# gitvicky/CP-PRE

Measured on AMD Instinct MI355X. Metric: residual-cells/s (PRE eval+calibrate), higher is better.
Workload: dtype f32

## Files before the change

### cp_pre_amd/csrc/calib.hip

```cpp
#include "common.h"

#pragma clang fp contract(off)

namespace {

__global__ void __launch_bounds__(256) absdiff_kernel(const float *__restrict__ a, const float *__restrict__ b,
                                                      float *__restrict__ out, long long n)
{
    const bool vec = !(((uintptr_t)a | (uintptr_t)out | (uintptr_t)(b ? b : a)) & 15);
    long long done = 0;
    if (vec) {
        const long long n4 = n / 4;
        const float4 *a4 = reinterpret_cast<const float4 *>(a);
        const float4 *b4 = reinterpret_cast<const float4 *>(b);
        float4 *o4 = reinterpret_cast<float4 *>(out);
        for (long long blk = blockIdx.x; blk * 1024 < n4; blk += gridDim.x) {
            const long long i = blk * 1024 + threadIdx.x;
            float4 v[4], w[4];
#pragma unroll
            for (int u = 0; u < 4; ++u)
                if (i + u * 256 < n4) v[u] = a4[i + u * 256];
            if (b) {
#pragma unroll
                for (int u = 0; u < 4; ++u)
                    if (i + u * 256 < n4) {
                        w[u] = b4[i + u * 256];
                        v[u] = make_float4(v[u].x - w[u].x, v[u].y - w[u].y, v[u].z - w[u].z, v[u].w - w[u].w);
                    }
            }
#pragma unroll
            for (int u = 0; u < 4; ++u)
                if (i + u * 256 < n4) o4[i + u * 256] = make_float4(fabsf(v[u].x), fabsf(v[u].y), fabsf(v[u].z), fabsf(v[u].w));
        }
        done = n4 * 4;
    }
    const long long stride = (long long)gridDim.x * blockDim.x;
    const long long tid = (long long)blockIdx.x * blockDim.x + threadIdx.x;
    for (long long i = done + tid; i < n; i += stride) out[i] = fabsf(b ? a[i] - b[i] : a[i]);
}

__global__ void __launch_bounds__(256) std_axis0_kernel(const float *__restrict__ a, const float *__restrict__ b,
                                                        int n, long long M, float eps, float *__restrict__ mod)
{
    const long long c = (long long)blockIdx.x * blockDim.x + threadIdx.x;
    if (c >= M) return;
    const float *pa = a + c, *pb = b ? b + c : nullptr;
    float s = 0.f;
#pragma unroll 16
    for (int i = 0; i < n; ++i) {
        const float v = pb ? pa[(long long)i * M] - pb[(long long)i * M] : pa[(long long)i * M];
        s = s + v;
    }
    const float mean = s / (float)n;
    float acc = 0.f;
#pragma unroll 16
    for (int i = 0; i < n; ++i) {
        const float v = pb ? pa[(long long)i * M] - pb[(long long)i * M] : pa[(long long)i * M];
        const float d = v - mean;
        const float dd = d * d;
        acc = acc + dd;
    }
    mod[c] = sqrtf(acc / (float)n) + eps;
}

__global__ void __launch_bounds__(256) moments_kernel(const float *__restrict__ a, const float *__restrict__ b,
                                                      int n, long long M, long long ld, int rows_per_split,
                                                      double *__restrict__ sum, double *__restrict__ sumsq)
{
    const long long c = (long long)blockIdx.x * blockDim.x + threadIdx.x;
    if (c >= M) return;
    const int i0 = blockIdx.y * rows_per_split;
    const int i1 = min(n, i0 + rows_per_split);
    double s = 0.0, q = 0.0;
#pragma unroll 8
    for (int i = i0; i < i1; ++i) {
        float v = a[(long long)i * ld + c];
        if (b) v = v - b[(long long)i * ld + c];
        const double d = (double)v;
        s += d;
        q += d * d;
    }
    if (gridDim.y == 1) { sum[c] += s; sumsq[c] += q; }
    else { atomicAdd(&sum[c], s); atomicAdd(&sumsq[c], q); }
}

constexpr int MS_TMAX = 16;
#ifndef MS_WANT1
#define MS_WANT1 1024
#endif
#ifndef MS_STAGE
#define MS_STAGE 1
#endif
__device__ __forceinline__ unsigned int wave_max_u32_to_lane63(unsigned int v)
{
#define PRE_DPP_MAX(ctrl, rows)                                                                                                 \
    v = max(v, (unsigned int)__builtin_amdgcn_update_dpp(0, (int)v, ctrl, rows, 0xf, true))
    PRE_DPP_MAX(0x111, 0xf);
    PRE_DPP_MAX(0x112, 0xf);
    PRE_DPP_MAX(0x114, 0xf);
    PRE_DPP_MAX(0x118, 0xf);
    PRE_DPP_MAX(0x142, 0xa);
    PRE_DPP_MAX(0x143, 0xc);
#undef PRE_DPP_MAX
    return v;
}

template <int O>
__device__ __forceinline__ unsigned int dpp_xor(unsigned int x)
{
    if constexpr (O == 1) return (unsigned int)__builtin_amdgcn_update_dpp(0, (int)x, 0xB1, 0xf, 0xf, true);
    else if constexpr (O == 2) return (unsigned int)__builtin_amdgcn_update_dpp(0, (int)x, 0x4E, 0xf, 0xf, true);
    else if constexpr (O == 8) return (unsigned int)__builtin_amdgcn_update_dpp(0, (int)x, 0x128, 0xf, 0xf, true);
    else {
        const int t = __builtin_amdgcn_update_dpp(0, (int)x, 0x104, 0xf, 0x5, false);
        return (unsigned int)__builtin_amdgcn_update_dpp(t, (int)x, 0x114, 0xf, 0xa, false);
    }
}

typedef unsigned int ms_u32x2 __attribute__((ext_vector_type(2)));
template <int US, int H>
__device__ __forceinline__ void ms_butterfly(unsigned int (&m)[US], int lane)
{
    if constexpr (H >= 1) {
        constexpr int width = 64 * H / US;
#pragma unroll
        for (int k = 0; k < H; ++k) {
            if constexpr (width == 32) {
                const ms_u32x2 r = __builtin_amdgcn_permlane32_swap(m[k], m[H + k], false, false);
                m[k] = max(r.x, r.y);
            } else if constexpr (width == 16) {
                const ms_u32x2 r = __builtin_amdgcn_permlane16_swap(m[k], m[H + k], false, false);
                m[k] = max(r.x, r.y);
            } else {
                const bool up = lane & width;
                const unsigned int mine = up ? m[H + k] : m[k], send = up ? m[k] : m[H + k];
                m[k] = max(mine, dpp_xor<width>(send));
            }
        }
        ms_butterfly<US, H / 2>(m, lane);
    }
}

__device__ __forceinline__ float ms_cell(const float *p, unsigned int cb, unsigned int plane_bytes)
{
    const __amdgpu_buffer_rsrc_t r = __builtin_amdgcn_make_buffer_rsrc(const_cast<float *>(p), 0, plane_bytes, 0x00020000);
    return __uint_as_float(__builtin_amdgcn_raw_buffer_load_b32(r, (int)cb, 0, 0));
}

template <int TCH, int US, bool FULL>
__device__ __forceinline__ void ms_load(const float *__restrict__ au, unsigned int c, long long row_stride, long long plane, int i, int nt,
                                        float (&v)[US][TCH])
{
#pragma unroll
    for (int u = 0; u < US; ++u)
#pragma unroll
        for (int t = 0; t < TCH; ++t)
            v[u][t] = ms_cell(au + ((i + u) * row_stride + (FULL || TCH == 1 || t < nt ? t : nt - 1) * plane), c, (unsigned int)plane * 4u);
}

struct MsStage { unsigned int (*m)[17]; unsigned int *row0; long long nseg_left; };
template <int TCH, int US, bool FULL>
__device__ __forceinline__ void ms_use(const float (&v)[US][TCH], int i, int nt, bool scored, double (&s)[TCH], double (&q)[TCH],
                                       unsigned int *__restrict__ seg, long long seg_stride, const MsStage *stage = nullptr)
{
    unsigned int m[US];
#pragma unroll
    for (int u = 0; u < US; ++u) {
        int mp = 0;
        unsigned int mn = 0u;
#pragma unroll
        for (int t = 0; t < TCH; ++t) {
            const float x = (FULL || TCH == 1 || t < nt) ? v[u][t] : 0.f;
            const double d = (double)x;
            s[t] += d;
            q[t] = __builtin_fma(d, d, q[t]);
            mp = max(mp, (int)__float_as_uint(x));
            mn = max(mn, __float_as_uint(x));
        }
        m[u] = max((unsigned int)mp, mn & 0x7fffffffu);
        m[u] = scored ? m[u] : 0u;
    }
    const int lane = threadIdx.x & 63;
    if constexpr (US == 1) {
        m[0] = wave_max_u32_to_lane63(m[0]);
        if (lane == 63 && seg) seg[i * seg_stride] = m[0];
    } else {
        ms_butterfly<US, US / 2>(m, lane);
        if constexpr (64 / US > 8) m[0] = max(m[0], dpp_xor<8>(m[0]));
        if constexpr (64 / US > 4) m[0] = max(m[0], dpp_xor<4>(m[0]));
        m[0] = max(m[0], dpp_xor<2>(m[0]));
        m[0] = max(m[0], dpp_xor<1>(m[0]));
        if (US == 16 && stage) {
            if ((lane & 3) == 0) stage->m[threadIdx.x >> 6][lane >> 2] = m[0];
            __syncthreads();
            if (threadIdx.x < 256) {
                const int smp = (int)(threadIdx.x >> 4), sg = (int)(threadIdx.x & 15);
                if (sg < stage->nseg_left) stage->row0[(i + smp) * seg_stride + sg] = stage->m[sg][smp];
            }
            __syncthreads();
        } else if ((lane & (64 / US - 1)) == 0) seg[(i + lane / (64 / US)) * seg_stride] = m[0];
    }
}

template <int TCH, int US, bool FULL>
__device__ __forceinline__ void ms_samples(const float *__restrict__ au, unsigned int c, long long row_stride, long long plane, int i0, int i1,
                                           int nt, bool scored, double (&s)[TCH], double (&q)[TCH], unsigned int *__restrict__ seg,
                                           long long seg_stride, const MsStage *stage = nullptr)
{
    int i = i0;
    if constexpr (US == 1) {
        float va[1][TCH], vb[1][TCH];
        if (i < i1) ms_load<TCH, 1, FULL>(au, c, row_stride, plane, i, nt, va);
        for (; i < i1; i += 2) {
            ms_load<TCH, 1, FULL>(au, c, row_stride, plane, min(i + 1, i1 - 1), nt, vb);
            ms_use<TCH, 1, FULL>(va, i, nt, scored, s, q, seg, seg_stride);
            if (i + 1 >= i1) break;
            ms_load<TCH, 1, FULL>(au, c, row_stride, plane, min(i + 2, i1 - 1), nt, va);
            ms_use<TCH, 1, FULL>(vb, i + 1, nt, scored, s, q, seg, seg_stride);
        }
    } else {
        float v[US][TCH], w[US][TCH], v1[1][TCH];
        const int ilast = i0 + (i1 - i0) / US * US - US;
        if (i + US <= i1) ms_load<TCH, US, FULL>(au, c, row_stride, plane, i, nt, v);
        for (; i + US <= i1; i += 2 * US) {
            ms_load<TCH, US, FULL>(au, c, row_stride, plane, min(i + US, ilast), nt, w);
            ms_use<TCH, US, FULL>(v, i, nt, scored, s, q, seg, seg_stride, stage);
            if (i + 2 * US > i1) { i += US; break; }
            ms_load<TCH, US, FULL>(au, c, row_stride, plane, min(i + 2 * US, ilast), nt, v);
            ms_use<TCH, US, FULL>(w, i + US, nt, scored, s, q, seg, seg_stride, stage);
        }
        for (; i < i1; ++i) {
            ms_load<TCH, 1, FULL>(au, c, row_stride, plane, i, nt, v1);
            ms_use<TCH, 1, FULL>(v1, i, nt, scored, s, q, seg, seg_stride);
        }
    }
}

template <int TCH, int US>
__global__ void __launch_bounds__(US == 16 && MS_STAGE ? 1024 : 256)
moments_segmax_kernel(const float *__restrict__ a, long long row_stride, int n, int T, int X,
                                                             int Y, int cx, int cy, int rows_per_split, double *__restrict__ sum,
                                                             double *__restrict__ sumsq, unsigned int *__restrict__ segmax)
{
    const long long plane = (long long)X * Y, cl = (long long)blockIdx.x * blockDim.x + threadIdx.x;
    if (!(US == 16 && MS_STAGE) && (cl & ~63LL) >= plane) return;
    const bool live = cl < plane;
    const long long c = live ? cl : plane - 1;
    const int x = (int)(c / Y), y = (int)(c - (long long)x * Y);
    const long long nseg = (plane + 63) / 64;
    const bool scored = live && x >= cx && x < X - cx && y >= cy && y < Y - cy;
    const int i0 = blockIdx.y * rows_per_split, i1 = min(n, i0 + rows_per_split);
    const int tc = blockIdx.z, TC = gridDim.z, t0 = tc * MS_TMAX, nt = min(TCH, T - t0);
    const float *au = a + (long long)t0 * plane;
    const long long seg_stride = (long long)TC * nseg;
    unsigned int *seg = segmax + (long long)tc * nseg + (cl >> 6);
    double s[TCH], q[TCH];
#pragma unroll
    for (int t = 0; t < TCH; ++t) s[t] = q[t] = 0.0;
    const unsigned int cb = (unsigned int)c * 4u;
    __shared__ unsigned int stage_m[US == 16 ? 16 : 1][17];
    MsStage st{stage_m, segmax + (long long)tc * nseg + (long long)blockIdx.x * (blockDim.x >> 6),
               nseg - (long long)blockIdx.x * (blockDim.x >> 6)};
    const MsStage *stage = (US == 16 && MS_STAGE) ? &st : nullptr;
    if (US == 16 && MS_STAGE && (cl & ~63LL) >= plane) seg = nullptr;
    if (nt == TCH) ms_samples<TCH, US, true>(au, cb, row_stride, plane, i0, i1, nt, scored, s, q, seg, seg_stride, stage);
    else ms_samples<TCH, US, false>(au, cb, row_stride, plane, i0, i1, nt, scored, s, q, seg, seg_stride, stage);
    sum += (long long)t0 * plane + c;
    sumsq += (long long)t0 * plane + c;
#pragma unroll
    for (int t = 0; t < TCH; ++t)
        if (t < nt && live) {
            if (gridDim.y == 1) { sum[t * plane] += s[t]; sumsq[t * plane] += q[t]; }
            else { atomicAdd(&sum[t * plane], s[t]); atomicAdd(&sumsq[t * plane], q[t]); }
        }
}

__global__ void __launch_bounds__(256) std_from_moments_kernel(const double *__restrict__ sum, const double *__restrict__ sumsq,
                                                               double n_total, long long M, float eps, float *__restrict__ mod)
{
    const long long c = (long long)blockIdx.x * blockDim.x + threadIdx.x;
    if (c >= M) return;
    const double mean = sum[c] / n_total;
    double var = sumsq[c] / n_total - mean * mean;
    var = var < 0.0 ? 0.0 : var;
    mod[c] = (float)sqrt(var) + eps;
}

__device__ __forceinline__ float wave_max(float v)
{
#pragma unroll
    for (int o = 32; o > 0; o >>= 1) v = fmaxf(v, __shfl_xor(v, o));
    return v;
}

constexpr int JS_RB = 32;
#ifndef JS_TARGET_CELLS
#define JS_TARGET_CELLS 65536
#endif
__device__ __forceinline__ void js_update(float av, float sv, float &m, float &thr, bool &nan)
{
    if (!(av <= thr * sv) || sv < 1.17549435e-38f) {
        const float q = av / sv;
        if (q != q) nan = true;
        else if (q > m) { m = q; thr = m * 0.99999905f; }
    }
}

__global__ void __launch_bounds__(256) joint_score_kernel(const float *__restrict__ a, const float *__restrict__ b,
                                                          const float *__restrict__ mod, int T, int X, int Y,
                                                          int ct, int cx, int cy, int groups, int smp_fastest,
                                                          const unsigned int *__restrict__ only, float *__restrict__ scores)
{
    const long long plane = (long long)X * Y, vol = plane * T;
    const int smp = smp_fastest ? blockIdx.x : blockIdx.y;
    const unsigned int cblk = smp_fastest ? blockIdx.y : blockIdx.x;
    if (only && !only[smp]) return;
    const float *pa = a + smp * vol, *pb = b ? b + smp * vol : nullptr;
    const long long nrows = (long long)T * X;
    const bool vec = (Y % 4 == 0) && !(((uintptr_t)a | (uintptr_t)mod | (uintptr_t)(b ? b : a)) & 15);
    __shared__ unsigned int rowmask;
    __shared__ float red[4];
    float m = 0.f, thr = 0.f;
    bool any = false, nan = false;
    for (int gi = 0; gi < groups; ++gi) {
    const long long r0 = ((long long)cblk * groups + gi) * JS_RB;
    if (r0 >= nrows) break;
    __syncthreads();
    if (threadIdx.x < 64) {
        const long long r = r0 + threadIdx.x;
        bool ok = threadIdx.x < JS_RB && r < nrows;
        if (ok) {
            const int t = (int)(r / X), x = (int)(r % X);
            ok = !(t < ct || t >= T - ct || x < cx || x >= X - cx);
        }
        const unsigned long long bm = __ballot(ok);
        if (threadIdx.x == 0) rowmask = (unsigned int)bm;
    }
    __syncthreads();
    const unsigned int rows = rowmask;
    any = any || rows != 0u;
    if (rows && vec) {
        const int Y4 = Y / 4, dr = 256 / Y4, dy = 256 % Y4;
        int row = threadIdx.x / Y4, y4 = threadIdx.x % Y4;
        while (row < JS_RB) {
            if ((rows >> row) & 1u) {
                const long long o = (r0 + row) * Y + 4 * y4;
                float4 v = *reinterpret_cast<const float4 *>(pa + o);
                if (pb) { const float4 w = *reinterpret_cast<const float4 *>(pb + o); v = make_float4(v.x - w.x, v.y - w.y, v.z - w.z, v.w - w.w); }
                const float4 sg = *reinterpret_cast<const float4 *>(mod + o);
                const float av[4] = {fabsf(v.x), fabsf(v.y), fabsf(v.z), fabsf(v.w)};
                const float sv[4] = {sg.x, sg.y, sg.z, sg.w};
                const int y = 4 * y4;
#pragma unroll
                for (int k = 0; k < 4; ++k)
                    if (y + k >= cy && y + k < Y - cy) js_update(av[k], sv[k], m, thr, nan);
            }
            y4 += dy;
            row += dr;
            if (y4 >= Y4) { y4 -= Y4; ++row; }
        }
    } else if (rows) {
        const int dr = 256 / Y, dy = 256 % Y;
        int row = threadIdx.x / Y, y = threadIdx.x % Y;
        while (row < JS_RB) {
            if (((rows >> row) & 1u) && y >= cy && y < Y - cy) {
                const long long o = (r0 + row) * Y + y;
                float v = pa[o];
                if (pb) v -= pb[o];
                js_update(fabsf(v), mod[o], m, thr, nan);
            }
            y += dy;
            row += dr;
            if (y >= Y) { y -= Y; ++row; }
        }
    }
    }
    m = wave_max(m);
    if (__ballot(nan)) m = __uint_as_float(0x7fc00000u);
    if ((threadIdx.x & 63) == 0) red[threadIdx.x >> 6] = m;
    __syncthreads();
    if (threadIdx.x == 0 && any) {
        const unsigned int u = max(max(__float_as_uint(red[0]), __float_as_uint(red[1])),
                                   max(__float_as_uint(red[2]), __float_as_uint(red[3])));
        atomicMax(reinterpret_cast<unsigned int *>(scores) + smp, u);
    }
}

constexpr int JSF_CELLS = 8192;
__global__ void __launch_bounds__(256) joint_score_flat_kernel(const float *__restrict__ a, const float *__restrict__ b,
                                                               const float *__restrict__ mod, int T, int X, int Y, int ct,
                                                               int cx, int cy, const unsigned int *__restrict__ only,
                                                               float *__restrict__ scores)
{
    const long long vol = (long long)T * X * Y;
    const int smp = blockIdx.x;
    if (only && !only[smp]) return;
    const float4 *pa = reinterpret_cast<const float4 *>(a + smp * vol);
    const float4 *pb = b ? reinterpret_cast<const float4 *>(b + smp * vol) : nullptr;
    const float4 *pm = reinterpret_cast<const float4 *>(mod);
    const unsigned int c0 = blockIdx.y * (unsigned)JSF_CELLS;
    __shared__ float red[4];
    float m = 0.f, thr = 0.f;
    bool nan = false;
    unsigned int f = c0 + 4u * threadIdx.x;
    const unsigned int row0 = f / (unsigned)Y;
    int y0 = (int)(f - row0 * (unsigned)Y), x0 = (int)(row0 % (unsigned)X), t0 = (int)(row0 / (unsigned)X);
    const int dy = 1024 % Y, drow = 1024 / Y, dx = drow % X, dt = drow / X;
    for (int k = 0; k < JSF_CELLS / 1024 && f < (unsigned)vol; ++k, f += 1024u) {
        float4 v = pa[f >> 2];
        if (pb) { const float4 w = pb[f >> 2]; v = make_float4(v.x - w.x, v.y - w.y, v.z - w.z, v.w - w.w); }
        const float4 sg = pm[f >> 2];
        const float av[4] = {fabsf(v.x), fabsf(v.y), fabsf(v.z), fabsf(v.w)};
        const float sv[4] = {sg.x, sg.y, sg.z, sg.w};
        int y = y0, x = x0, t = t0;
#pragma unroll
        for (int j = 0; j < 4; ++j) {
            const bool in = t >= ct && t < T - ct && x >= cx && x < X - cx && y >= cy && y < Y - cy;
            if (in) js_update(av[j], sv[j], m, thr, nan);
            if (++y == Y) { y = 0; if (++x == X) { x = 0; ++t; } }
        }
        y0 += dy;
        const int carry = y0 >= Y;
        y0 -= carry ? Y : 0;
        x0 += dx + carry;
        const int cx2 = x0 >= X;
        x0 -= cx2 ? X : 0;
        t0 += dt + cx2;
    }
    m = wave_max(m);
    if (__ballot(nan)) m = __uint_as_float(0x7fc00000u);
    if ((threadIdx.x & 63) == 0) red[threadIdx.x >> 6] = m;
    __syncthreads();
    if (threadIdx.x == 0) {
        const unsigned int u = max(max(__float_as_uint(red[0]), __float_as_uint(red[1])),
                                   max(__float_as_uint(red[2]), __float_as_uint(red[3])));
        if (u) atomicMax(reinterpret_cast<unsigned int *>(scores) + smp, u);
    }
}

constexpr int JP_SEG = 64;

__global__ void __launch_bounds__(64) segmin_kernel(const float *__restrict__ mod, int T, int X, int Y, int cx, int cy,
                                                    long long nseg, float *__restrict__ segmin)
{
    const long long plane = (long long)X * Y, seg = blockIdx.x, c = seg * JP_SEG + (long long)threadIdx.x;
    const int tc = blockIdx.y, x = (int)(c / Y), y = (int)(c - (long long)x * Y);
    float m = __builtin_inff();
    bool bad = false;
    if (c < plane && x >= cx && x < X - cx && y >= cy && y < Y - cy)
        for (int t = tc * MS_TMAX; t < min(T, (tc + 1) * MS_TMAX); ++t) {
            const float v = mod[t * plane + c];
            bad |= !(v > 0.f);
            m = fminf(m, v);
        }
#pragma unroll
    for (int o = 32; o > 0; o >>= 1) m = fminf(m, __shfl_xor(m, o));
    bad = __ballot(bad) != 0;
    if (threadIdx.x == 0) segmin[(long long)tc * nseg + seg] = bad ? 0.f : m;
}

template <bool WAVE>
__global__ void __launch_bounds__(1024) joint_score_pruned_kernel(const float *__restrict__ res, long long row_stride,
                                                                  const float *__restrict__ mod,
                                                                  const unsigned int *__restrict__ segmax,
                                                                  const float *__restrict__ segmin, int n, int T, int X, int Y, int cx,
                                                                  int cy, int per_chunk, int total, float *__restrict__ scores,
                                                                  unsigned int *__restrict__ flags,
                                                                  unsigned long long *__restrict__ stats)
{
    extern __shared__ unsigned int work_all[];
    __shared__ unsigned int red[16], redi[16], nwork_[4], sbest_[4], blk_read, blk_flagged;
    const int lane = threadIdx.x & 63;
    const int wave = WAVE ? 0 : (int)(threadIdx.x >> 6), nwaves = WAVE ? 1 : (int)(blockDim.x >> 6);
    const int mywave = (int)(threadIdx.x >> 6);
    const int tid = WAVE ? lane : (int)threadIdx.x, nthreads = WAVE ? 64 : (int)blockDim.x;
    const int smp = WAVE ? (int)blockIdx.x * 4 + mywave : (int)blockIdx.x;
    unsigned int *work = work_all + (WAVE ? mywave * total : 0);
    unsigned int &nwork = nwork_[WAVE ? mywave : 0], &sbest = sbest_[WAVE ? mywave : 0];
    auto sync = [&]() __attribute__((always_inline)) {
        if constexpr (WAVE) {
            __builtin_amdgcn_fence(__ATOMIC_RELEASE, "wavefront");
            __builtin_amdgcn_wave_barrier();
            __builtin_amdgcn_fence(__ATOMIC_ACQUIRE, "wavefront");
        } else {
            __syncthreads();
        }
    };
    if (WAVE && threadIdx.x == 0) { blk_read = 0u; blk_flagged = 0u; }
    if (WAVE) __syncthreads();
    unsigned int my_read = 0u, my_flagged = 0u;
    do {
    if (WAVE && smp >= n) break;
    const float *pr = res + smp * row_stride;
    const unsigned int *pm = segmax + (long long)smp * total;
    const long long plane = (long long)X * Y;
    const unsigned int NANBITS = 0x7fc00000u;

    auto bound = [&](int j) __attribute__((always_inline)) {
        const float sm = segmin[j];
        if (sm == 0.f) return NANBITS;
        const unsigned int mx = pm[j];
        if (mx == 0u) return 0u;
        const float q = __uint_as_float(mx) / sm;
        return q != q ? NANBITS : __float_as_uint(q);
    };
    auto evaluate = [&](int j) __attribute__((always_inline)) {
        const int tc = j / per_chunk;
        const long long c = (long long)(j - tc * per_chunk) * JP_SEG + lane;
        const int x = (int)(c / Y), y = (int)(c - (long long)x * Y);
        const int t0 = tc * MS_TMAX, planes = min(MS_TMAX, T - t0);
        unsigned int m = 0u;
        if (c < plane && x >= cx && x < X - cx && y >= cy && y < Y - cy) {
            const long long o = (long long)t0 * plane + c;
            float rv[MS_TMAX], mv[MS_TMAX];
#pragma unroll
            for (int t = 0; t < MS_TMAX; ++t) {
                const int tt = t < planes ? t : planes - 1;
                rv[t] = pr[o + tt * plane];
                mv[t] = mod[o + tt * plane];
            }
#pragma unroll
            for (int t = 0; t < MS_TMAX; ++t) {
                const float q = fabsf(rv[t]) / mv[t];
                m = max(m, q != q ? NANBITS : (q > 0.f ? __float_as_uint(q) : 0u));
            }
        }
#pragma unroll
        for (int o = 32; o > 0; o >>= 1) m = max(m, (unsigned int)__shfl_xor((int)m, o));
        return m;
    };

    unsigned int bb = 0u, bj = 0u;
    for (int j = tid; j < total; j += nthreads) {
        const unsigned int b = bound(j);
        if (b > bb) { bb = b; bj = (unsigned)j; }
    }
#pragma unroll
    for (int o = 32; o > 0; o >>= 1) {
        const unsigned int ob = (unsigned int)__shfl_xor((int)bb, o), oj = (unsigned int)__shfl_xor((int)bj, o);
        if (ob > bb || (ob == bb && oj < bj)) { bb = ob; bj = oj; }
    }
    if (!WAVE && lane == 0) { red[wave] = bb; redi[wave] = bj; }
    if (tid == 0) nwork = 0u;
    sync();
    if (!WAVE) {
        bb = red[0], bj = redi[0];
        for (int w = 1; w < nwaves; ++w)
            if (red[w] > bb || (red[w] == bb && redi[w] < bj)) { bb = red[w]; bj = redi[w]; }
    }
    unsigned int best = __float_as_uint(scores[smp]);
    if (bb == 0u) {
        if (flags && tid == 0) flags[smp] = 0u;
        break;
    }
    if (bb > best) best = max(best, evaluate((int)bj));
    for (int j = tid; j < total; j += nthreads)
        if ((unsigned)j != bj && bound(j) > best) work[atomicAdd(&nwork, 1u)] = (unsigned)j;
    if (tid == 0) sbest = best;
    sync();
    const unsigned int nw = nwork;
    {
        const bool giveup = flags && 4u * nw > (unsigned)total;
        my_read = giveup ? (unsigned)total : nw + 1u;
        my_flagged = giveup ? 1u : 0u;
    }
    if (flags) {
        const bool giveup = 4u * nw > (unsigned)total;
        if (tid == 0) flags[smp] = giveup ? 1u : 0u;
        if (giveup) {
            if (tid == 0) atomicMax(reinterpret_cast<unsigned int *>(scores) + smp, best);
            break;
        }
    }
    for (unsigned int i = wave; i < nw; i += nwaves) {
        const int j = (int)work[i];
        best = max(best, *(volatile unsigned int *)&sbest);
        if (bound(j) > best) {
            const unsigned int v = evaluate(j);
            if (v > best) { best = v; if (lane == 0) atomicMax(&sbest, v); }
        }
    }
    sync();
    if (tid == 0) atomicMax(reinterpret_cast<unsigned int *>(scores) + smp, max(best, sbest));
    } while (false);
    if (!stats) return;
    if (blockIdx.x == 0 && threadIdx.x == 0) atomicAdd(&stats[1], (unsigned long long)n * (unsigned long long)total);
    if constexpr (WAVE) {
        if (lane == 0 && my_read) atomicAdd(&blk_read, my_read);
        if (lane == 0 && my_flagged) atomicAdd(&blk_flagged, my_flagged);
        __syncthreads();
        if (threadIdx.x == 0) {
            if (blk_read) atomicAdd(&stats[0], (unsigned long long)blk_read);
            if (blk_flagged) atomicAdd(&stats[2], (unsigned long long)blk_flagged);
        }
    } else if (threadIdx.x == 0) {
        if (my_read) atomicAdd(&stats[0], (unsigned long long)my_read);
        if (my_flagged) atomicAdd(&stats[2], 1ull);
    }
}

struct KList { int nk; long long k[16]; };

__global__ void __launch_bounds__(1024) kth_kernel(const float *__restrict__ s, long long N, const KList kl, float *__restrict__ out)
{
    __shared__ unsigned int hist[256];
    __shared__ unsigned int sh_prefix;
    __shared__ long long sh_rank;
    __shared__ int sh_nan;
    const int j = blockIdx.x;
    const int lane = threadIdx.x & 63;
    unsigned int prefix = 0, mask = 0;
    long long rank = kl.k[j];
    if (threadIdx.x == 0) sh_nan = 0;
    const bool vec = !((uintptr_t)s & 15);
    const long long N8 = vec ? N / 8 : 0;
    for (int shift = 24; shift >= 0; shift -= 8) {
        if (threadIdx.x < 256) hist[threadIdx.x] = 0;
        __syncthreads();
        auto count = [&](float v) __attribute__((always_inline)) {
            if (shift == 24 && v != v) sh_nan = 1;
            const unsigned int key = f2key(v);
            const bool hit = (key & mask) == prefix;
            const unsigned int d = (key >> shift) & 255u;
            const unsigned long long hm = __ballot(hit);
            if (hm) {
                const int first = __builtin_ctzll(hm);
                const unsigned int d0 = __builtin_amdgcn_readlane((int)d, first);
                if (__ballot(hit && d == d0) == hm) {
                    if (lane == first) atomicAdd(&hist[d0], (unsigned)__popcll(hm));
                } else if (hit) {
                    atomicAdd(&hist[d], 1u);
                }
            }
        };
        const float4 *s4 = reinterpret_cast<const float4 *>(s);
        for (long long i = threadIdx.x; i < N8; i += blockDim.x) {
            const float4 a = s4[2 * i], b = s4[2 * i + 1];
            count(a.x); count(a.y); count(a.z); count(a.w);
            count(b.x); count(b.y); count(b.z); count(b.w);
        }
        for (long long i = 8 * N8 + threadIdx.x; i < N; i += blockDim.x) count(s[i]);
        __syncthreads();
        if (threadIdx.x < 64) {
            const unsigned int c0 = hist[4 * lane], c1 = hist[4 * lane + 1], c2 = hist[4 * lane + 2], c3 = hist[4 * lane + 3];
            long long incl = (long long)c0 + c1 + c2 + c3;
#pragma unroll
            for (int o = 1; o < 64; o <<= 1) {
                const long long up = __shfl_up(incl, o);
                if (lane >= o) incl += up;
            }
            long long excl = incl - ((long long)c0 + c1 + c2 + c3);
            const bool mine = (excl <= rank && rank < incl) || (lane == 63 && rank >= incl);
            if (mine) {
                unsigned int d = 4 * lane;
                if (rank >= excl + c0) { excl += c0; ++d; if (rank >= excl + c1) { excl += c1; ++d; if (rank >= excl + c2) { excl += c2; ++d; } } }
                sh_prefix = prefix | (d << shift);
                sh_rank = rank - excl;
            }
        }
        __syncthreads();
        prefix = sh_prefix;
        rank = sh_rank;
        mask |= 255u << shift;
        __syncthreads();
    }
    if (threadIdx.x == 0) out[j] = sh_nan ? __uint_as_float(0x7fc00000u) : key2f(prefix);
}

__global__ void __launch_bounds__(256) cov_count_kernel(const float *__restrict__ y, const float *__restrict__ lo,
                                                        const float *__restrict__ hi, long long total, long long M,
                                                        int per_sample, unsigned long long *count)
{
    unsigned int local = 0;
    for (long long i = (long long)blockIdx.x * blockDim.x + threadIdx.x; i < total; i += (long long)gridDim.x * blockDim.x) {
        const long long c = per_sample ? i : i % M;
        const float v = y[i];
        local += (v >= lo[c]) && (v <= hi[c]);
    }
#pragma unroll
    for (int o = 32; o > 0; o >>= 1) local += __shfl_xor(local, o);
    __shared__ unsigned int red[4];
    if ((threadIdx.x & 63) == 0) red[threadIdx.x >> 6] = local;
    __syncthreads();
    if (threadIdx.x == 0) atomicAdd(count, (unsigned long long)(red[0] + red[1] + red[2] + red[3]));
}

__global__ void __launch_bounds__(256) cov_count4_kernel(const float4 *__restrict__ y, const float4 *__restrict__ lo,
                                                         const float4 *__restrict__ hi, int n, long long M4, int per_sample,
                                                         int rows_per, unsigned long long *count)
{
    const long long q = (long long)blockIdx.x * blockDim.x + threadIdx.x;
    unsigned int local = 0;
    if (q < M4) {
        const int s0 = blockIdx.y * rows_per, s1 = min(n, s0 + rows_per);
        float4 l = lo[q], h = hi[q];
        auto inside = [&](const float4 &v, const float4 &a, const float4 &b) __attribute__((always_inline)) {
            return (unsigned)((v.x >= a.x) && (v.x <= b.x)) + (unsigned)((v.y >= a.y) && (v.y <= b.y)) +
                   (unsigned)((v.z >= a.z) && (v.z <= b.z)) + (unsigned)((v.w >= a.w) && (v.w <= b.w));
        };
        int s = s0;
        if (!per_sample) {
            for (; s + 7 < s1; s += 8) {
                float4 v[8];
#pragma unroll
                for (int u = 0; u < 8; ++u) v[u] = y[(long long)(s + u) * M4 + q];
#pragma unroll
                for (int u = 0; u < 8; ++u) local += inside(v[u], l, h);
            }
        }
        for (; s < s1; ++s) {
            const long long o = (long long)s * M4 + q;
            if (per_sample) { l = lo[o]; h = hi[o]; }
            local += inside(y[o], l, h);
        }
    }
#pragma unroll
    for (int o = 32; o > 0; o >>= 1) local += __shfl_xor(local, o);
    __shared__ unsigned int red[4];
    if ((threadIdx.x & 63) == 0) red[threadIdx.x >> 6] = local;
    __syncthreads();
    if (threadIdx.x == 0 && (red[0] | red[1] | red[2] | red[3])) atomicAdd(count, (unsigned long long)(red[0] + red[1] + red[2] + red[3]));
}

__global__ void __launch_bounds__(256) cov_joint_kernel(const float *__restrict__ y, const float *__restrict__ lo,
                                                        const float *__restrict__ hi, long long M, int per_sample,
                                                        uint8_t *inside)
{
    const int smp = blockIdx.y;
    const float *py = y + smp * M;
    const float *plo = lo + (per_sample ? smp * M : 0), *phi = hi + (per_sample ? smp * M : 0);
    bool bad = false;
    if (M % 4 == 0 && !(((uintptr_t)y | (uintptr_t)lo | (uintptr_t)hi) & 15)) {
        const float4 *y4 = reinterpret_cast<const float4 *>(py), *l4 = reinterpret_cast<const float4 *>(plo),
                     *h4 = reinterpret_cast<const float4 *>(phi);
        for (long long q = (long long)blockIdx.x * blockDim.x + threadIdx.x; q < M / 4; q += (long long)gridDim.x * blockDim.x) {
            const float4 v = y4[q], a = l4[q], b = h4[q];
            bad |= !((v.x >= a.x) && (v.x <= b.x) && (v.y >= a.y) && (v.y <= b.y) && (v.z >= a.z) && (v.z <= b.z) &&
                     (v.w >= a.w) && (v.w <= b.w));
        }
    } else {
        for (long long c = (long long)blockIdx.x * blockDim.x + threadIdx.x; c < M; c += (long long)gridDim.x * blockDim.x) {
            const float v = py[c];
            bad |= !((v >= plo[c]) && (v <= phi[c]));
        }
    }
    if (__any(bad) && (threadIdx.x & 63) == 0) inside[smp] = 0;
}

__global__ void __launch_bounds__(256) cov_rowcount_kernel(const float *__restrict__ y, const float *__restrict__ lo,
                                                           const float *__restrict__ hi, long long M, int per_sample,
                                                           int outside, unsigned int *__restrict__ counts)
{
    const int smp = blockIdx.y;
    const float *py = y + smp * M;
    const float *plo = lo + (per_sample ? smp * M : 0), *phi = hi + (per_sample ? smp * M : 0);
    unsigned int local = 0;
    auto hit = [&](float v, float a, float b) __attribute__((always_inline)) {
        return (unsigned)(outside ? ((v <= a) || (v >= b)) : ((v >= a) && (v <= b)));
    };
    if (M % 4 == 0 && !(((uintptr_t)y | (uintptr_t)lo | (uintptr_t)hi) & 15)) {
        const float4 *y4 = reinterpret_cast<const float4 *>(py), *l4 = reinterpret_cast<const float4 *>(plo),
                     *h4 = reinterpret_cast<const float4 *>(phi);
        for (long long q = (long long)blockIdx.x * blockDim.x + threadIdx.x; q < M / 4; q += (long long)gridDim.x * blockDim.x) {
            const float4 v = y4[q], a = l4[q], b = h4[q];
            local += hit(v.x, a.x, b.x) + hit(v.y, a.y, b.y) + hit(v.z, a.z, b.z) + hit(v.w, a.w, b.w);
        }
    } else {
        for (long long c = (long long)blockIdx.x * blockDim.x + threadIdx.x; c < M; c += (long long)gridDim.x * blockDim.x)
            local += hit(py[c], plo[c], phi[c]);
    }
#pragma unroll
    for (int o = 32; o > 0; o >>= 1) local += __shfl_xor(local, o);
    if ((threadIdx.x & 63) == 0 && local) atomicAdd(counts + smp, local);
}

inline unsigned grid_for(long long items, int block, long long cap = 256LL * 32)
{
    long long g = (items + block - 1) / block;
    if (g < 1) g = 1;
    return (unsigned)(g > cap ? cap : g);
}

}

extern "C" {

int pre_absdiff_f32(const float *a, const float *b, float *out, int64_t n, void *stream)
{
    if (!a || !out || n < 0) return PRE_E_NULL;
    if (n == 0) return PRE_OK;
    hipLaunchKernelGGL(absdiff_kernel, dim3(grid_for(n / 16 + 1, 256, 0x7fffffffLL)), dim3(256), 0, as_stream(stream), a, b, out, (long long)n);
    PRE_LAUNCH_CHECK();
    return PRE_OK;
}

int pre_std_axis0_f32(const float *a, const float *b, int64_t n, int64_t M, float eps, float *mod, void *stream)
{
    if (!a || !mod || n <= 0 || M <= 0) return PRE_E_NULL;
    if (n > 0x7fffffff || M > 0xffffff00LL) return PRE_E_SHAPE;
    const int bs = M >= (1 << 19) ? 256 : 64;
    hipLaunchKernelGGL(std_axis0_kernel, dim3((unsigned)((M + bs - 1) / bs)), dim3(bs), 0, as_stream(stream), a, b, (int)n,
                       (long long)M, eps, mod);
    PRE_LAUNCH_CHECK();
    return PRE_OK;
}

int pre_moments_axis0_f64(const float *a, const float *b, int64_t n, int64_t M, int64_t row_stride, double *sum,
                          double *sumsq, void *stream)
{
    if (!a || !sum || !sumsq || n <= 0 || M <= 0 || row_stride < M) return PRE_E_NULL;
    if (n > 0x7fffffff || M > 0xffffff00LL) return PRE_E_SHAPE;
    const long long bx = (M + 255) / 256;
    long long splits = 1;
    while (bx * splits < 1024 && splits * 32 < n) splits *= 2;
    const int rows = (int)((n + splits - 1) / splits);
    splits = (n + rows - 1) / rows;
    hipLaunchKernelGGL(moments_kernel, dim3((unsigned)bx, (unsigned)splits), dim3(256), 0, as_stream(stream), a, b, (int)n,
                       (long long)M, (long long)row_stride, rows, sum, sumsq);
    PRE_LAUNCH_CHECK();
    return PRE_OK;
}

int pre_moments_segmax_f64(const float *a, int64_t row_stride, int64_t n, int64_t T, int64_t X, int64_t Y, int crop_x, int crop_y,
                           double *sum, double *sumsq, uint32_t *segmax, void *stream)
{
    if (!a || !sum || !sumsq || !segmax || n <= 0 || T <= 0 || X <= 0 || Y <= 0) return PRE_E_NULL;
    if (crop_x < 0 || crop_y < 0 || row_stride < T * X * Y) return PRE_E_RANGE;
    const int us = T == 1 ? 16 : T <= 4 ? 4 : 1;
    const int bt = (us == 16 && MS_STAGE) ? 1024 : 256;
    const long long bx = (X * Y + bt - 1) / bt, TC = (T + MS_TMAX - 1) / MS_TMAX;
    if (n > 0x7fffffff || bx > 0x7fffffffLL || TC > 65535 || T > 0x7fffffff) return PRE_E_SHAPE;
    if (X * Y >= (1LL << 30)) return PRE_E_SHAPE;
    long long splits = 1;
    const long long want = us == 16 ? 16384 : us > 1 ? 2048 : MS_WANT1;
    while (bx * (bt / 256) * TC * splits < want && splits * 32 * us < n) splits *= 2;
    const int rows = (int)((n + splits - 1) / splits);
    splits = (n + rows - 1) / rows;
    const dim3 grid((unsigned)bx, (unsigned)splits, (unsigned)TC);
#define PRE_MS_LAUNCH(TCH, US)                                                                                                \
    hipLaunchKernelGGL((moments_segmax_kernel<TCH, US>), grid, dim3(bt), 0, as_stream(stream), a, (long long)row_stride, (int)n,    \
                       (int)T, (int)X, (int)Y, crop_x, crop_y, rows, sum, sumsq, segmax)
    if (us == 16) PRE_MS_LAUNCH(1, 16);
    else if (us == 4) PRE_MS_LAUNCH(4, 4);
    else PRE_MS_LAUNCH(MS_TMAX, 1);
#undef PRE_MS_LAUNCH
    PRE_LAUNCH_CHECK();
    return PRE_OK;
}

int pre_std_from_moments_f32(const double *sum, const double *sumsq, int64_t n_total, int64_t M, float eps, float *mod,
                             void *stream)
{
    if (!sum || !sumsq || !mod || n_total <= 0 || M <= 0) return PRE_E_NULL;
    if (M > 0xffffff00LL) return PRE_E_SHAPE;
    hipLaunchKernelGGL(std_from_moments_kernel, dim3((unsigned)((M + 255) / 256)), dim3(256), 0, as_stream(stream), sum, sumsq,
                       (double)n_total, (long long)M, eps, mod);
    PRE_LAUNCH_CHECK();
    return PRE_OK;
}

static int joint_score_launch(const float *a, const float *b, const float *mod, int64_t n, int64_t T, int64_t X, int64_t Y,
                              int crop_t, int crop_x, int crop_y, const uint32_t *only, float *scores, void *stream)
{
    if (!a || !mod || !scores || n <= 0 || T <= 0 || X <= 0 || Y <= 0) return PRE_E_NULL;
    if (crop_t < 0 || crop_x < 0 || crop_y < 0) return PRE_E_RANGE;
    if (n > 65535 * 1024LL || T * X > 0x7fffffffLL * JS_RB || Y > 0x7fffffff) return PRE_E_SHAPE;
    {
        const long long vol = (long long)T * X * Y, nblk = (vol + JSF_CELLS - 1) / JSF_CELLS;
        if (Y < 64 && vol % 4 == 0 && vol < 0x7fffffffLL && nblk <= 65535 && n <= 0x7fffffff &&
            !(((uintptr_t)a | (uintptr_t)mod | (uintptr_t)(b ? b : a)) & 15)) {
            hipLaunchKernelGGL(joint_score_flat_kernel, dim3((unsigned)n, (unsigned)nblk), dim3(256), 0, as_stream(stream), a, b, mod,
                               (int)T, (int)X, (int)Y, crop_t, crop_x, crop_y, only, scores);
            PRE_LAUNCH_CHECK();
            return PRE_OK;
        }
    }
    const long long spans = (T * X + JS_RB - 1) / JS_RB;
    long long groups = JS_TARGET_CELLS / (JS_RB * Y);
    if (groups < 1) groups = 1;
    while (groups > 1 && (spans / groups) * n < 2048) groups /= 2;
    const long long chunks = (spans + groups - 1) / groups;
    for (int64_t s0 = 0; s0 < n; s0 += 65535) {
        const int64_t ns = (n - s0) < 65535 ? (n - s0) : 65535;
        const long long vol = (long long)T * X * Y;
        const int swap = chunks <= 65535;
        hipLaunchKernelGGL(joint_score_kernel, swap ? dim3((unsigned)ns, (unsigned)chunks) : dim3((unsigned)chunks, (unsigned)ns),
                           dim3(256), 0, as_stream(stream), a + s0 * vol, b ? b + s0 * vol : nullptr, mod, (int)T, (int)X, (int)Y,
                           crop_t, crop_x, crop_y, (int)groups, swap, only ? only + s0 : nullptr, scores + s0);
        PRE_LAUNCH_CHECK();
    }
    return PRE_OK;
}

int pre_joint_score_f32(const float *a, const float *b, const float *mod, int64_t n, int64_t T, int64_t X, int64_t Y,
                        int crop_t, int crop_x, int crop_y, float *scores, void *stream)
{
    return joint_score_launch(a, b, mod, n, T, X, Y, crop_t, crop_x, crop_y, nullptr, scores, stream);
}

int pre_joint_score_flagged_f32(const float *a, const float *b, const float *mod, int64_t n, int64_t T, int64_t X, int64_t Y,
                                int crop_t, int crop_x, int crop_y, const uint32_t *flags, float *scores, void *stream)
{
    if (!flags) return PRE_E_NULL;
    return joint_score_launch(a, b, mod, n, T, X, Y, crop_t, crop_x, crop_y, flags, scores, stream);
}

int pre_segmin_mod_f32(const float *mod, int64_t T, int64_t X, int64_t Y, int crop_x, int crop_y, float *segmin, void *stream)
{
    if (!mod || !segmin || T <= 0 || X <= 0 || Y <= 0) return PRE_E_NULL;
    if (crop_x < 0 || crop_y < 0) return PRE_E_RANGE;
    const long long nseg = (X * Y + JP_SEG - 1) / JP_SEG, TC = (T + MS_TMAX - 1) / MS_TMAX;
    if (X > 0x7fffffff || Y > 0x7fffffff || nseg > 0x7fffffffLL || TC > 65535) return PRE_E_SHAPE;
    hipLaunchKernelGGL(segmin_kernel, dim3((unsigned)nseg, (unsigned)TC), dim3(64), 0, as_stream(stream), mod, (int)T, (int)X, (int)Y,
                       crop_x, crop_y, nseg, segmin);
    PRE_LAUNCH_CHECK();
    return PRE_OK;
}

static int pruned_lds_max()
{
    int dev = 0, lds_max = 0;
    if (hipGetDevice(&dev) != hipSuccess ||
        hipDeviceGetAttribute(&lds_max, hipDeviceAttributeMaxSharedMemoryPerBlock, dev) != hipSuccess || lds_max <= 0) {
        (void)hipGetLastError();
        lds_max = 64 * 1024;
    }
    return lds_max;
}

int64_t pre_joint_score_pruned_max_segments(void) { return (pruned_lds_max() - 256) / 4; }

int pre_joint_score_pruned_f32(const float *res, int64_t row_stride, const float *mod, const uint32_t *segmax, const float *segmin,
                               int64_t n, int64_t T, int64_t X, int64_t Y, int crop_x, int crop_y, float *scores,
                               uint32_t *flags, unsigned long long *stats, void *stream)
{
    if (!res || !mod || !segmax || !segmin || !scores || n <= 0 || T <= 0 || X <= 0 || Y <= 0) return PRE_E_NULL;
    if (crop_x < 0 || crop_y < 0 || row_stride < T * X * Y) return PRE_E_RANGE;
    const long long nseg = (X * Y + JP_SEG - 1) / JP_SEG, TC = (T + MS_TMAX - 1) / MS_TMAX, total = TC * nseg;
    if (n > 0x7fffffff || T > 0x7fffffff || X > 0x7fffffff || Y > 0x7fffffff) return PRE_E_SHAPE;
    const int lds_max = pruned_lds_max();
    if (total * 4 + 256 > lds_max) return PRE_E_UNSUPPORTED;
    if (total * 4 + 256 > 64 * 1024) {
        if (hipFuncSetAttribute(reinterpret_cast<const void *>(joint_score_pruned_kernel<false>), hipFuncAttributeMaxDynamicSharedMemorySize,
                                lds_max - 256) != hipSuccess) {
            (void)hipGetLastError();
            return PRE_E_UNSUPPORTED;
        }
    }
    if (n >= 4096 && total <= 2048) {
        hipLaunchKernelGGL(joint_score_pruned_kernel<true>, dim3((unsigned)((n + 3) / 4)), dim3(256), (size_t)total * 16,
                           as_stream(stream), res, (long long)row_stride, mod, segmax, segmin, (int)n, (int)T, (int)X, (int)Y, crop_x,
                           crop_y, (int)nseg, (int)total, scores, flags, stats);
        PRE_LAUNCH_CHECK();
        return PRE_OK;
    }
    const int threads = n >= 2048 ? 256 : n >= 512 ? 512 : 1024;
    hipLaunchKernelGGL(joint_score_pruned_kernel<false>, dim3((unsigned)n), dim3(threads), (size_t)total * 4, as_stream(stream), res,
                       (long long)row_stride, mod, segmax, segmin, (int)n, (int)T, (int)X, (int)Y, crop_x, crop_y, (int)nseg, (int)total,
                       scores, flags, stats);
    PRE_LAUNCH_CHECK();
    return PRE_OK;
}

int pre_kth_f32(const float *scores, int64_t N, const int64_t *ks, int nk, float *out, void *stream)
{
    if (!scores || !ks || !out || N <= 0 || nk <= 0) return PRE_E_NULL;
    for (int j = 0; j < nk; ++j)
        if (ks[j] < 0 || ks[j] >= N) return PRE_E_RANGE;
    for (int j0 = 0; j0 < nk; j0 += 16) {
        KList kl;
        kl.nk = (nk - j0) < 16 ? (nk - j0) : 16;
        for (int j = 0; j < kl.nk; ++j) kl.k[j] = ks[j0 + j];
        hipLaunchKernelGGL(kth_kernel, dim3(kl.nk), dim3(1024), 0, as_stream(stream), scores, (long long)N, kl, out + j0);
        PRE_LAUNCH_CHECK();
    }
    return PRE_OK;
}

int pre_cov_count_f32(const float *y, const float *lo, const float *hi, int64_t n, int64_t M, int per_sample_bounds,
                      unsigned long long *count, void *stream)
{
    if (!y || !lo || !hi || !count || n <= 0 || M <= 0) return PRE_E_NULL;
    if (M % 4 == 0 && !(((uintptr_t)y | (uintptr_t)lo | (uintptr_t)hi) & 15) && n <= 0x7fffffff) {
        const long long M4 = M / 4, bx = (M4 + 255) / 256;
        long long groups = (4096 + bx - 1) / bx;
        long long rows_per = (n + groups - 1) / groups;
        rows_per = (rows_per + 7) / 8 * 8;
        groups = (n + rows_per - 1) / rows_per;
        if (bx <= 0x7fffffffLL && groups <= 65535) {
            hipLaunchKernelGGL(cov_count4_kernel, dim3((unsigned)bx, (unsigned)groups), dim3(256), 0, as_stream(stream),
                               reinterpret_cast<const float4 *>(y), reinterpret_cast<const float4 *>(lo),
                               reinterpret_cast<const float4 *>(hi), (int)n, M4, per_sample_bounds, (int)rows_per, count);
            PRE_LAUNCH_CHECK();
            return PRE_OK;
        }
    }
    hipLaunchKernelGGL(cov_count_kernel, dim3(grid_for(n * M, 256)), dim3(256), 0, as_stream(stream), y, lo, hi,
                       (long long)(n * M), (long long)M, per_sample_bounds, count);
    PRE_LAUNCH_CHECK();
    return PRE_OK;
}

int pre_cov_rowcount_f32(const float *y, const float *lo, const float *hi, int64_t n, int64_t M, int per_sample_bounds,
                         int outside, uint32_t *counts, void *stream)
{
    if (!y || !lo || !hi || !counts || n <= 0 || M <= 0) return PRE_E_NULL;
    const unsigned gx = grid_for(M, 256, 64);
    for (int64_t s0 = 0; s0 < n; s0 += 65535) {
        const int64_t ns = (n - s0) < 65535 ? (n - s0) : 65535;
        hipLaunchKernelGGL(cov_rowcount_kernel, dim3(gx, (unsigned)ns), dim3(256), 0, as_stream(stream), y + s0 * M,
                           per_sample_bounds ? lo + s0 * M : lo, per_sample_bounds ? hi + s0 * M : hi, (long long)M,
                           per_sample_bounds, outside, counts + s0);
        PRE_LAUNCH_CHECK();
    }
    return PRE_OK;
}

int pre_cov_joint_f32(const float *y, const float *lo, const float *hi, int64_t n, int64_t M, int per_sample_bounds,
                      uint8_t *inside, void *stream)
{
    if (!y || !lo || !hi || !inside || n <= 0 || M <= 0) return PRE_E_NULL;
    const unsigned gx = grid_for(M, 256, 64);
    for (int64_t s0 = 0; s0 < n; s0 += 65535) {
        const int64_t ns = (n - s0) < 65535 ? (n - s0) : 65535;
        hipLaunchKernelGGL(cov_joint_kernel, dim3(gx, (unsigned)ns), dim3(256), 0, as_stream(stream), y + s0 * M,
                           per_sample_bounds ? lo + s0 * M : lo, per_sample_bounds ? hi + s0 * M : hi, (long long)M,
                           per_sample_bounds, inside + s0);
        PRE_LAUNCH_CHECK();
    }
    return PRE_OK;
}

}
```

Baseline: 289.6 billion.

## Add vectorized 1024-thread moments+segmax kernel for T>4 with LDS-staged segment max

Adds a new moments/segmax kernel for the multi-timestep case (T>4) that has each thread load four consecutive cells as 128-bit buffer loads for four timesteps. Loads are double-buffered across samples, and segment maxima are reduced with DPP row shifts and staged in double-buffered shared memory before one barrier per group of samples. The goal is fewer memory instructions, better load latency hiding and fewer per-sample syncs than the scalar 256-thread path. In exchange it raises register pressure (16 double accumulators per moment) and uses a different split heuristic. It only applies when the plane size and row stride are multiples of four and the input is 16-byte aligned.

New measurement: 297.7 billion (median of 6 runs). 1.03x the previous value.

```diff
diff --git a/cp_pre_amd/csrc/calib.hip b/cp_pre_amd/csrc/calib.hip
--- a/cp_pre_amd/csrc/calib.hip
+++ b/cp_pre_amd/csrc/calib.hip
@@ -272,6 +272,136 @@
         if (t < nt && live) {
             if (gridDim.y == 1) { sum[t * plane] += s[t]; sumsq[t * plane] += q[t]; }
             else { atomicAdd(&sum[t * plane], s[t]); atomicAdd(&sumsq[t * plane], q[t]); }
+        }
+}
+
+constexpr int MS4_US = 8;
+constexpr int MS4_CG = 4;
+constexpr int MS4_NT = 256 * MS4_CG, MS4_NW = 4 * MS4_CG;
+constexpr int MS4_WANT = 256;
+constexpr int MS4_AUX = 2;
+typedef unsigned int ms4_u32x4 __attribute__((ext_vector_type(4)));
+
+__device__ __forceinline__ void ms4_barrier()
+{
+    __builtin_amdgcn_fence(__ATOMIC_RELEASE, "workgroup", "local");
+    __builtin_amdgcn_s_barrier();
+    __builtin_amdgcn_fence(__ATOMIC_ACQUIRE, "workgroup", "local");
+}
+
+__device__ __forceinline__ void ms4_load(const float *au, unsigned int cb, long long row_stride, long long plane, int i, int nt,
+                                         ms4_u32x4 (&v)[4])
+{
+#pragma unroll
+    for (int k = 0; k < 4; ++k) {
+        const __amdgpu_buffer_rsrc_t r = __builtin_amdgcn_make_buffer_rsrc(
+            const_cast<float *>(au + ((long long)i * row_stride + k * plane)), 0, k < nt ? (unsigned int)plane * 4u : 0u, 0x00020000);
+        v[k] = __builtin_amdgcn_raw_buffer_load_b128(r, (int)cb, 0, MS4_AUX);
+    }
+}
+
+__device__ __forceinline__ unsigned int ms4_use(const ms4_u32x4 (&v)[4], const bool (&scored)[4], double (&s)[4][4], double (&q)[4][4])
+{
+    unsigned int m = 0u;
+#pragma unroll
+    for (int j = 0; j < 4; ++j) {
+        int mp = 0;
+        unsigned int mn = 0u;
+#pragma unroll
+        for (int k = 0; k < 4; ++k) {
+            const unsigned int b = v[k][j];
+            const double d = (double)__uint_as_float(b);
+            s[k][j] += d;
+            q[k][j] = __builtin_fma(d, d, q[k][j]);
+            mp = max(mp, (int)b);
+            mn = max(mn, b);
+        }
+        const unsigned int mc = max((unsigned int)mp, mn & 0x7fffffffu);
+        m = max(m, scored[j] ? mc : 0u);
+    }
+    return m;
+}
+
+__device__ __forceinline__ void ms4_sample(const ms4_u32x4 (&v)[4], const bool (&scored)[4], double (&s)[4][4], double (&q)[4][4],
+                                           unsigned int (&slot)[MS4_NW][4], int w, int lane)
+{
+    unsigned int m = ms4_use(v, scored, s, q);
+    m = max(m, (unsigned int)__builtin_amdgcn_update_dpp(0, (int)m, 0x111, 0xf, 0xf, true));
+    m = max(m, (unsigned int)__builtin_amdgcn_update_dpp(0, (int)m, 0x112, 0xf, 0xf, true));
+    m = max(m, (unsigned int)__builtin_amdgcn_update_dpp(0, (int)m, 0x114, 0xf, 0xf, true));
+    m = max(m, (unsigned int)__builtin_amdgcn_update_dpp(0, (int)m, 0x118, 0xf, 0xf, true));
+    if ((lane & 15) == 15) slot[w][lane >> 4] = m;
+}
+
+__device__ __forceinline__ void ms4_samples(const float *au, unsigned int cb, long long row_stride, long long plane, int i0, int i1,
+                                            int nt, const bool (&scored)[4], double (&s)[4][4], double (&q)[4][4],
+                                            unsigned int (*stage)[MS4_US][MS4_NW][4], unsigned int *row0, int nseg_left,
+                                            long long seg_stride)
+{
+    const int w = __builtin_amdgcn_readfirstlane((int)(threadIdx.x >> 6)), lane = (int)(threadIdx.x & 63);
+    ms4_u32x4 va[4], vb[4];
+    ms4_load(au, cb, row_stride, plane, i0, nt, va);
+    int b = 0;
+    for (int ib = i0; ib < i1; ib += MS4_US, b ^= 1) {
+        const int cnt = min(MS4_US, i1 - ib);
+#pragma unroll
+        for (int u = 0; u < MS4_US; u += 2) {
+            ms4_load(au, cb, row_stride, plane, min(ib + u + 1, i1 - 1), nt, vb);
+            if (u < cnt) ms4_sample(va, scored, s, q, stage[b][u], w, lane);
+            ms4_load(au, cb, row_stride, plane, min(ib + u + 2, i1 - 1), nt, va);
+            if (u + 1 < cnt) ms4_sample(vb, scored, s, q, stage[b][u + 1], w, lane);
+        }
+        ms4_barrier();
+        if (threadIdx.x < MS4_US * MS4_NW) {
+            const int smp = (int)(threadIdx.x / MS4_NW), sg = (int)(threadIdx.x % MS4_NW), cg = sg >> 2, r = sg & 3;
+            const unsigned int m = max(max(stage[b][smp][4 * cg][r], stage[b][smp][4 * cg + 1][r]),
+                                       max(stage[b][smp][4 * cg + 2][r], stage[b][smp][4 * cg + 3][r]));
+            if (smp < cnt && sg < nseg_left) row0[(long long)(ib + smp) * seg_stride + sg] = m;
+        }
+    }
+}
+
+__global__ void __launch_bounds__(MS4_NT) moments_segmax4_kernel(const float *__restrict__ a, long long row_stride, int n, int T,
+                                                               int X, int Y, int cx, int cy, int rows_per_split,
+                                                               double *__restrict__ sum, double *__restrict__ sumsq,
+                                                               unsigned int *__restrict__ segmax)
+{
+    const long long plane = (long long)X * Y;
+    const int w = __builtin_amdgcn_readfirstlane((int)(threadIdx.x >> 6)), lane = (int)(threadIdx.x & 63);
+    const long long cl = (long long)blockIdx.x * MS4_NT + (w >> 2) * 256 + lane * 4;
+    const bool live = cl < plane;
+    const long long c = live ? cl : plane - 4;
+    bool scored[4];
+#pragma unroll
+    for (int j = 0; j < 4; ++j) {
+        const int x = (int)((c + j) / Y), y = (int)(c + j - (long long)x * Y);
+        scored[j] = live && x >= cx && x < X - cx && y >= cy && y < Y - cy;
+    }
+    const long long nseg = (plane + 63) / 64;
+    const int i0 = blockIdx.y * rows_per_split, i1 = min(n, i0 + rows_per_split);
+    const int tc = blockIdx.z, TC = gridDim.z, t0 = tc * MS_TMAX + 4 * (w & 3), nt = min(4, T - t0);
+    const float *au = a + (long long)min(t0, T - 1) * plane;
+    const long long seg_stride = (long long)TC * nseg;
+    unsigned int *row0 = segmax + (long long)tc * nseg + (long long)blockIdx.x * MS4_NW;
+    const int nseg_left = (int)min((long long)MS4_NW, nseg - (long long)blockIdx.x * MS4_NW);
+    double s[4][4], q[4][4];
+#pragma unroll
+    for (int k = 0; k < 4; ++k)
+#pragma unroll
+        for (int j = 0; j < 4; ++j) s[k][j] = q[k][j] = 0.0;
+    __shared__ unsigned int stage[2][MS4_US][MS4_NW][4];
+    const unsigned int cb = (unsigned int)c * 4u;
+    ms4_samples(au, cb, row_stride, plane, i0, i1, nt, scored, s, q, stage, row0, nseg_left, seg_stride);
+    if (!live) return;
+#pragma unroll
+    for (int k = 0; k < 4; ++k)
+        if (k < nt) {
+            double *ps = sum + (long long)(t0 + k) * plane + c, *pq = sumsq + (long long)(t0 + k) * plane + c;
+#pragma unroll
+            for (int j = 0; j < 4; ++j) {
+                if (gridDim.y == 1) { ps[j] += s[k][j]; pq[j] += q[k][j]; }
+                else { atomicAdd(&ps[j], s[k][j]); atomicAdd(&pq[j], q[k][j]); }
+            }
         }
 }
 
@@ -827,6 +957,20 @@
     if (!a || !sum || !sumsq || !segmax || n <= 0 || T <= 0 || X <= 0 || Y <= 0) return PRE_E_NULL;
     if (crop_x < 0 || crop_y < 0 || row_stride < T * X * Y) return PRE_E_RANGE;
     const int us = T == 1 ? 16 : T <= 4 ? 4 : 1;
+    if (us == 1 && (X * Y) % 4 == 0 && row_stride % 4 == 0 && !((uintptr_t)a & 15)) {
+        const long long bx = (X * Y + MS4_NT - 1) / MS4_NT, TC = (T + MS_TMAX - 1) / MS_TMAX;
+        if (n > 0x7fffffff || bx > 0x7fffffffLL || TC > 65535 || T > 0x7fffffff) return PRE_E_SHAPE;
+        if (X * Y >= (1LL << 30)) return PRE_E_SHAPE;
+        long long splits = 1;
+        while (bx * TC * splits < MS4_WANT && splits * 32 < n) splits *= 2;
+        const int rows = (int)((n + splits - 1) / splits);
+        splits = (n + rows - 1) / rows;
+        hipLaunchKernelGGL(moments_segmax4_kernel, dim3((unsigned)bx, (unsigned)splits, (unsigned)TC), dim3(MS4_NT), 0,
+                           as_stream(stream), a, (long long)row_stride, (int)n, (int)T, (int)X, (int)Y, crop_x, crop_y, rows, sum,
+                           sumsq, segmax);
+        PRE_LAUNCH_CHECK();
+        return PRE_OK;
+    }
     const int bt = (us == 16 && MS_STAGE) ? 1024 : 256;
     const long long bx = (X * Y + bt - 1) / bt, TC = (T + MS_TMAX - 1) / MS_TMAX;
     if (n > 0x7fffffff || bx > 0x7fffffffLL || TC > 65535 || T > 0x7fffffff) return PRE_E_SHAPE;
```
